# choyingw/SynergyNet

Measured on NVIDIA H100. Metric: faces/sec (120x120, batch 1024 per GPU, backbone + 3DMM params + 68 landmarks), higher is better.
Workload: dtype f32

## Files before the change

### synergynet_b200/csrc/kernels_fused.cuh

```cuda
#pragma once
#include "common.cuh"
#include "tc_common.cuh"

namespace syn {

constexpr int kFusedWorkerWarps = 8;
static_assert(kFusedWorkerWarps % 4 == 0, "worker warps form whole warpgroups");

__host__ __device__ constexpr int ceil_div_c(int a, int b) { return (a + b - 1) / b; }
__host__ __device__ constexpr int round_up_c(int a, int b) { return ceil_div_c(a, b) * b; }

template <int CIN_, int CHID_, int NC_, int COUT_, int W_, int STRIDE_, int RO_, int FACES_, bool RES_, bool STEM_,
          int WSTREAM_>
struct FusedCfg {
  static constexpr bool STEM = STEM_;
  static constexpr bool RES = RES_;
  static constexpr bool WSTREAM = WSTREAM_ > 0;
  static constexpr int CIN = CIN_;
  static constexpr int CIN_P = round_up_c(CIN_, 16);
  static constexpr int CHID = CHID_, NC = NC_, NCHUNK = CHID_ / NC_;
  static constexpr int COUT = COUT_, COUT_P = round_up_c(COUT_, 16);
  static constexpr int W = W_, STRIDE = STRIDE_, WO = (W_ - 1) / STRIDE_ + 1;
  static constexpr int RO = RO_, STRIPS = WO / RO_, FACES = FACES_;
  static constexpr int RWIN = (RO_ - 1) * STRIDE_ + 3;
  static constexpr int ROWS_MAX = (RWIN < W_ ? RWIN : W_);
  static constexpr int M1_MAX = FACES_ * ROWS_MAX * W_;
  static constexpr int MT1 = ceil_div_c(M1_MAX, 128);
  static constexpr int M2F = RO_ * WO;
  static constexpr int M2_MAX = FACES_ * M2F;
  static constexpr int MT2 = ceil_div_c(M2_MAX, 128);
  static constexpr int HS_COLS = W_ + 2;
  static constexpr int HS_FACE = RWIN * HS_COLS, HS_PIX = FACES_ * HS_FACE, HS_STRIDE = NC_ + 4;
  static constexpr int DWS = NC_ + 4;
  static constexpr int SLABS1 = ceil_div_c(M1_MAX, 64), SLABS2 = ceil_div_c(M2_MAX, 64);
  static constexpr int B3_BYTES = round_up_c(2 * COUT_P * 4, 128);
  static constexpr int W1_PLANE = NC_ * CIN_P * 2;
  static constexpr int W3_PLANE = COUT_P * NC_ * 2;
  static constexpr int DW_ROWS = 12;
  static constexpr int CH_W1 = 0, CH_W3 = 2 * W1_PLANE, CH_DW = CH_W3 + 2 * W3_PLANE;
  static constexpr int CHUNK_BYTES = round_up_c(CH_DW + DW_ROWS * DWS * 4, 128);
  static constexpr int W_BYTES = B3_BYTES + NCHUNK * CHUNK_BYTES;
  static constexpr int WSTAGES = WSTREAM_ > 0 ? WSTREAM_ : NCHUNK;
  static constexpr int A2_PLANE = MT2 * 128 * NC_ * 2;
  static constexpr int XA_TILE = 64 * CIN_P * 2, XA_PLANE = SLABS1 * XA_TILE;
  static constexpr int S_B3 = 0;
  static constexpr int S_WCH = S_B3 + B3_BYTES;
  static constexpr int S_XA = S_WCH + WSTAGES * CHUNK_BYTES;
  static constexpr int S_A2 = S_XA + 2 * XA_PLANE;
  static constexpr int S_H = S_A2 + 2 * A2_PLANE;
  static constexpr int IN_ROWS = 2 * ROWS_MAX + 1, IN_STRIDE = 120;
  static constexpr int S_IN = S_H + HS_PIX * HS_STRIDE * 4;
  static constexpr int S_TOTAL = S_IN + (STEM_ ? 3 * IN_ROWS * IN_STRIDE * 4 : 0);
  static constexpr int SMEM_BYTES = S_TOTAL + 1024;
  static_assert(CHID_ % NC_ == 0 && NC_ % 16 == 0, "hidden chunking");
  static_assert(WO % RO_ == 0, "strips must tile the output");
  static_assert(FACES_ == 1 || RO_ == WO, "multi-face tiles hold whole faces");
  static_assert(SMEM_BYTES <= 227 * 1024, "shared memory");
  static_assert(NC_ <= 256, "MMA N");
  static_assert(WSTREAM_ == 0 || (WSTREAM_ >= 2 && WSTREAM_ <= 4 && NCHUNK >= WSTREAM_), "weight ring");
};

struct FusedArgs {
  const float* x;
  const uint8_t* x_u8;
  const uint8_t* wimg;
  float* y;
  int batch;
  int split;
  int face_groups;
  int* err;
  int* sat;
  int border;
  int npass;
#ifdef SYN_FUSED_TRACE
  int trace_id;
#endif
};

#ifdef SYN_FUSED_TRACE
__device__ long long g_fused_trace[18 * 2 * 64 * 8];
#define SYN_TRACE(role, chunk, ev)                                                                        \
  do {                                                                                                    \
    if (trace_on) g_fused_trace[((p.trace_id * 2 + (role)) * 64 + (chunk)) * 8 + (ev)] = clock64();      \
  } while (0)
#else
#define SYN_TRACE(role, chunk, ev) do { } while (0)
#endif

template <int THREADS>
__device__ __forceinline__ void group_bar_sync(int grp) {
  switch (grp) {
    case 0: asm volatile("bar.sync 1, %0;" ::"n"(THREADS) : "memory"); break;
    case 1: asm volatile("bar.sync 2, %0;" ::"n"(THREADS) : "memory"); break;
    case 2: asm volatile("bar.sync 3, %0;" ::"n"(THREADS) : "memory"); break;
    default: asm volatile("bar.sync 4, %0;" ::"n"(THREADS) : "memory"); break;
  }
}

__host__ __device__ constexpr int fused_d2_pieces(int cout_p, int slabs, int nwg) {
  int s = 1;
  while (slabs * s < nwg && (cout_p / (2 * s)) % 8 == 0) s *= 2;
  return s;
}

template <int N, int KSTEPS, int NPASS>
__device__ __forceinline__ void fused_mma_group(float* acc, uint32_t d_hi, uint32_t a_lo, uint32_t a_plane, uint32_t a_kstep,
                                                uint32_t b_lo, uint32_t b_plane, uint32_t b_kstep, bool acc_in) {
  tc::wgmma_fence();
#pragma unroll
  for (int pass = 0; pass < NPASS; ++pass)
#pragma unroll
    for (int ks = 0; ks < KSTEPS; ++ks)
      tc::wgmma_f16<N>(acc, tc::desc64(d_hi, a_lo + (((pass == 2 ? a_plane : 0) + ks * a_kstep) >> 4)),
                       tc::desc64(d_hi, b_lo + (((pass == 1 ? b_plane : 0) + ks * b_kstep) >> 4)),
                       (acc_in || pass > 0 || ks > 0) ? 1u : 0u);
  tc::wgmma_commit();
}

template <class C>
__global__ void __launch_bounds__((kFusedWorkerWarps + 1) * 32, 1) fused_mbconv_kernel(const FusedArgs p) {
  constexpr int NWW = kFusedWorkerWarps;
  constexpr int NWT = NWW * 32;
  constexpr int NWG = NWW / 4;
  constexpr int NKG_ = C::NC / 8;
  constexpr int NG = 1;
  constexpr int WPG = NWW / NG, TPG = WPG * 32;
  constexpr int KPG = NKG_ / NG;
  constexpr int NSPL = fused_d2_pieces(C::COUT_P, C::SLABS2, NWG);
  constexpr int N2 = C::COUT_P / NSPL;
  constexpr int IPW = ceil_div_c(C::SLABS2 * NSPL, NWG);
  static_assert(N2 % 8 == 0 && N2 <= 256, "MMA N");
  using namespace tc;
  extern __shared__ __align__(1024) uint8_t smem_raw[];
  __shared__ __align__(8) uint64_t bar_w, bar_wfull[4], bar_wempty[4], bar_x, bar_in;

  uint8_t* smem = smem_raw + ((1024u - (smem_u32(smem_raw) & 1023u)) & 1023u);
  const int tid = threadIdx.x, warp = tid >> 5;
  const int row = tid & 127, wg = __shfl_sync(0xffffffffu, tid >> 7, 0);
  const int grp = warp / WPG;
  const int gtid = tid - grp * TPG;
  const int ntiles = p.face_groups * C::STRIPS;
  auto group_faces = [&](int fg, int& f0, int& nfaces) {
    if constexpr (C::FACES == 2) {
      if (fg < p.split) { f0 = 2 * fg; nfaces = 2; }
      else { f0 = 2 * p.split + (fg - p.split); nfaces = 1; }
    } else {
      f0 = fg * C::FACES;
      nfaces = min(C::FACES, p.batch - f0);
    }
  };

  asm volatile("griddepcontrol.launch_dependents;" ::: "memory");
  if (tid == 0) {
    mbar_init(smem_u32(&bar_w), 1);
    for (int i = 0; i < 4; ++i) {
      mbar_init(smem_u32(&bar_wfull[i]), 1);
      mbar_init(smem_u32(&bar_wempty[i]), NWT);
    }
    mbar_init(smem_u32(&bar_x), NWT);
    mbar_init(smem_u32(&bar_in), 1);
    fence_mbar_init();
  }
  if constexpr (C::STEM) {
    float* z = reinterpret_cast<float*>(smem_raw + ((1024u - (tc::smem_u32(smem_raw) & 1023u)) & 1023u) + C::S_IN);
    for (int i = threadIdx.x; i < 3 * C::IN_ROWS * C::IN_STRIDE / 4; i += blockDim.x)
      reinterpret_cast<float4*>(z)[i] = make_float4(0.f, 0.f, 0.f, 0.f);
    tc::fence_proxy_async_smem();
  }
  __syncthreads();

  uint8_t* sWch = smem + C::S_WCH;
  uint8_t* sXA = smem + C::S_XA;
  uint8_t* sA2 = smem + C::S_A2;
  float* sH = reinterpret_cast<float*>(smem + C::S_H);
  const float* sB3 = reinterpret_cast<const float*>(smem + C::S_B3);
  float* sIn = reinterpret_cast<float*>(smem + C::S_IN);

  if (warp < NWW) {
    for (int i = tid; i < C::HS_PIX * C::HS_STRIDE / 4; i += NWT)
      reinterpret_cast<float4*>(sH)[i] = make_float4(0.f, 0.f, 0.f, 0.f);
    mbar_wait(smem_u32(&bar_w), 0, p.err);
    uint32_t g = 0, n_in = 0;
    asm volatile("bar.sync 5, %0;" ::"n"(NWT) : "memory");
    const uint32_t d_hi = smem_desc_hi(128);
    constexpr uint32_t LBO_W1 = (C::NC / 8) * 128, LBO_W3 = (C::COUT_P / 8) * 128;

    constexpr int SPW = ceil_div_c(C::SLABS1, NWG);
    constexpr bool LATE_G1 = C::WSTREAM && C::WSTAGES == 2;
    auto issue_g1 = [&](bool on, float* acc, int s1, const uint8_t* wch) {
      if (on) {
        const uint32_t a_lo = smem_desc_lo(smem_u32(sXA + s1 * C::XA_TILE), 1024);
        const uint32_t w_lo = smem_desc_lo(smem_u32(wch + C::CH_W1), LBO_W1);
        if (p.npass == 1) fused_mma_group<C::NC, C::CIN_P / 16, 1>(acc, d_hi, a_lo, C::XA_PLANE, 2048, w_lo, C::W1_PLANE, 2 * LBO_W1, false);
        else fused_mma_group<C::NC, C::CIN_P / 16, 3>(acc, d_hi, a_lo, C::XA_PLANE, 2048, w_lo, C::W1_PLANE, 2 * LBO_W1, false);
      } else {
        wgmma_fence();
        wgmma_commit();
      }
    };

    auto prep = [&](int tile) {
      const int fg = tile / C::STRIPS, sp = tile - fg * C::STRIPS;
      int f0, nfaces;
      group_faces(fg, f0, nfaces);
      const int iy0 = sp * C::RO * C::STRIDE - 1;
      const int rf = max(iy0, 0), rl = min(iy0 + C::RWIN - 1, C::W - 1);
      const int ppf = (rl - rf + 1) * C::W;
      const int M1 = nfaces * ppf;
      const int mt1 = (M1 + 127) >> 7;
#ifdef SYN_FUSED_TRACE
      const bool trace_on = blockIdx.x == 0 && tile == 2 * (int)gridDim.x && tid == 0;
#endif
      SYN_TRACE(0, 62, 0);
      if constexpr (C::STEM) {
        const int iy_first = 2 * rf - 1, nin = 2 * (rl - rf + 1) + 1;
        if (p.x_u8 != nullptr) {
          for (int i = tid; i < 3 * nin * 30; i += NWT) {
            const int c4 = i % 30, r = (i / 30) % nin, ci = i / (30 * nin);
            const int iy = iy_first + r;
            float4 v = make_float4(0.f, 0.f, 0.f, 0.f);
            if (iy >= 0 && iy < kImg) {
              uchar4 u = *reinterpret_cast<const uchar4*>(p.x_u8 + ((size_t)(f0 * 3 + ci) * kImg + iy) * kImg + c4 * 4);
              if (p.border > 0) {
                const int col = c4 * 4;
                const bool row_out = iy < p.border || iy >= kImg - p.border;
                if (row_out || col < p.border || col >= kImg - p.border) u.x = 0;
                if (row_out || col + 1 < p.border || col + 1 >= kImg - p.border) u.y = 0;
                if (row_out || col + 2 < p.border || col + 2 >= kImg - p.border) u.z = 0;
                if (row_out || col + 3 < p.border || col + 3 >= kImg - p.border) u.w = 0;
              }
              v = make_float4(((float)u.x - 127.5f) / 128.0f, ((float)u.y - 127.5f) / 128.0f,
                              ((float)u.z - 127.5f) / 128.0f, ((float)u.w - 127.5f) / 128.0f);
            }
            *reinterpret_cast<float4*>(sIn + (ci * C::IN_ROWS + r) * C::IN_STRIDE + c4 * 4) = v;
          }
        } else {
          mbar_wait(smem_u32(&bar_in), n_in & 1, p.err);
          ++n_in;
          for (int r = 0; r < nin; ++r) {
            const int iy = iy_first + r;
            if (iy < 0 || iy >= kImg)
              for (int i = tid; i < 3 * 30; i += NWT)
                *reinterpret_cast<float4*>(sIn + ((i / 30) * C::IN_ROWS + r) * C::IN_STRIDE + (i % 30) * 4) =
                    make_float4(0.f, 0.f, 0.f, 0.f);
          }
        }
        SYN_TRACE(0, 62, 1);
        asm volatile("bar.sync 5, %0;" ::"n"(NWT) : "memory");
      }
      SYN_TRACE(0, 62, 2);
      {
        constexpr int KG = C::CIN_P / 8;
        constexpr int NXG = NWT / 64;
        constexpr int ITERS = (C::SLABS1 * KG + NXG - 1) / NXG;
        constexpr int PB = ITERS < 4 ? ITERS : 4;
        const int r64 = tid & 63, xg = tid >> 6;
        const int n_items = ((M1 + 63) >> 6) * KG;
        for (int e0 = xg; e0 < n_items; e0 += PB * NXG) {
          float v[PB][8];
          if constexpr (C::STEM) {
#pragma unroll
            for (int u = 0; u < PB; ++u) {
#pragma unroll
              for (int j = 0; j < 8; ++j) v[u][j] = 0.f;
              const int e = e0 + u * NXG;
              if (e >= n_items) continue;
              const int t = e / KG, kg = e - t * KG;
              const int mr = t * 64 + r64;
              if (mr < M1) {
                const int yl = mr / C::W, xx = mr - yl * C::W;
                const float* base = sIn + (2 * yl) * C::IN_STRIDE + 2 * xx - 1;
#pragma unroll
                for (int kgc = 0; kgc < KG; ++kgc)
                  if (kg == kgc) {
#pragma unroll
                    for (int j = 0; j < 8; ++j) {
                      const int k = kgc * 8 + j;
                      if (k < 27) {
                        const int ci = k / 9, ky = (k % 9) / 3, kx = k % 3;
                        if (kx > 0 || xx > 0) v[u][j] = base[(ci * C::IN_ROWS + ky) * C::IN_STRIDE + kx];
                      }
                    }
                  }
              }
            }
          } else {
            float4 qa[PB], qb[PB];
            bool ok[PB];
#pragma unroll
            for (int u = 0; u < PB; ++u) {
              const int e = min(e0 + u * NXG, n_items - 1);
              const int t = e / KG, kg = e - t * KG;
              const int m = t * 64 + r64;
              ok[u] = (e0 + u * NXG < n_items) && (m < M1) && (kg * 8 < C::CIN);
              const int mc = min(m, M1 - 1), kgc = min(kg, (C::CIN - 1) / 8);
              const int f = (C::FACES > 1) ? mc / ppf : 0;
              const int mr = mc - f * ppf;
              const float* src = p.x + ((size_t)((f0 + f) * C::W + rf) * C::W + mr) * C::CIN + kgc * 8;
              qa[u] = __ldg(reinterpret_cast<const float4*>(src));
              qb[u] = __ldg(reinterpret_cast<const float4*>(src + 4));
            }
            if (e0 == xg) SYN_TRACE(0, 62, 5);
#pragma unroll
            for (int u = 0; u < PB; ++u) {
              v[u][0] = ok[u] ? qa[u].x : 0.f; v[u][1] = ok[u] ? qa[u].y : 0.f; v[u][2] = ok[u] ? qa[u].z : 0.f; v[u][3] = ok[u] ? qa[u].w : 0.f;
              v[u][4] = ok[u] ? qb[u].x : 0.f; v[u][5] = ok[u] ? qb[u].y : 0.f; v[u][6] = ok[u] ? qb[u].z : 0.f; v[u][7] = ok[u] ? qb[u].w : 0.f;
            }
          }
#pragma unroll
          for (int u = 0; u < PB; ++u) {
            const int e = e0 + u * NXG;
            if (e < n_items) {
              const int t = e / KG, kg = e - t * KG;
              uint32_t h[4], l[4];
              float vmax = 0.f;
#pragma unroll
              for (int j = 0; j < 8; ++j) vmax = fmaxf(vmax, fabsf(v[u][j]));
              if (vmax * kActScale > 60000.f) *p.sat = 1;
#pragma unroll
              for (int j = 0; j < 4; ++j) split2_f16(v[u][2 * j] * kActScale, v[u][2 * j + 1] * kActScale, h[j], l[j]);
              uint8_t* xa = sXA + t * C::XA_TILE + (r64 >> 3) * 128 + kg * 1024 + (r64 & 7) * 16;
              *reinterpret_cast<uint4*>(xa) = make_uint4(h[0], h[1], h[2], h[3]);
              *reinterpret_cast<uint4*>(xa + C::XA_PLANE) = make_uint4(l[0], l[1], l[2], l[3]);
              if (e == xg) SYN_TRACE(0, 62, 6);
            }
          }
          if (e0 == xg) SYN_TRACE(0, 62, 7);
        }
      }
      SYN_TRACE(0, 62, 3);
      fence_proxy_async_smem();
      mbar_arrive(smem_u32(&bar_x));
      SYN_TRACE(0, 62, 4);

    };
    auto prefetch_x = [&](int tile) {
      if constexpr (!C::STEM) {
        if (tile >= ntiles) return;
        const int fg = tile / C::STRIPS, sp = tile - fg * C::STRIPS;
        int f0, nfaces;
        group_faces(fg, f0, nfaces);
        const int iy0 = sp * C::RO * C::STRIDE - 1;
        const int rf = max(iy0, 0), rl = min(iy0 + C::RWIN - 1, C::W - 1);
        const char* base = reinterpret_cast<const char*>(p.x + ((size_t)(f0 * C::W + rf) * C::W) * C::CIN);
        const int bytes = (C::FACES > 1 ? nfaces * C::W * C::W : (rl - rf + 1) * C::W) * C::CIN * 4;
        for (int o = tid * 128; o < bytes; o += NWT * 128)
          asm volatile("prefetch.global.L2 [%0];" ::"l"(base + o));
      }
    };
    asm volatile("griddepcontrol.wait;" ::: "memory");
    if ((int)blockIdx.x < ntiles) prep(blockIdx.x);
    prefetch_x(blockIdx.x + gridDim.x);

    for (int tile = blockIdx.x; tile < ntiles; tile += gridDim.x) {
      const int fg = tile / C::STRIPS, sp = tile - fg * C::STRIPS;
      int f0, nfaces;
      group_faces(fg, f0, nfaces);
      const int oy0 = sp * C::RO;
      const int iy0 = oy0 * C::STRIDE - 1;
      const int rf = max(iy0, 0), rl = min(iy0 + C::RWIN - 1, C::W - 1);
      const int ppf = (rl - rf + 1) * C::W;
#ifdef SYN_FUSED_TRACE
      const bool trace_on = blockIdx.x == 0 && tile == (int)gridDim.x && tid == 0;
#endif
      SYN_TRACE(0, 63, 0);
      const int M1 = nfaces * ppf;
      const int mt1 = (M1 + 127) >> 7;
      const int M2 = nfaces * C::M2F;
      const int mt2 = (M2 + 127) >> 7;

      const int slabs1 = (M1 + 63) >> 6;
      float acc1[2][C::NC / 2];
      float acc2[IPW][N2 / 2];
      auto chunk_slot = [&](uint32_t gc, int c) -> const uint8_t* {
        const int slot = C::WSTREAM ? (int)(gc % C::WSTAGES) : c;
        if constexpr (C::WSTREAM) mbar_wait(smem_u32(&bar_wfull[slot]), (gc / C::WSTAGES) & 1, p.err);
        return sWch + slot * C::CHUNK_BYTES;
      };
      auto gemm1_epi1 = [&](int c, const uint8_t* wch) {
        const float* dwc = reinterpret_cast<const float*>(wch + C::CH_DW);
        const float sc1 = dwc[11 * C::DWS];
        const float* b1 = dwc + 10 * C::DWS;
#pragma unroll
        for (int j = 0; j < SPW; ++j) {
          const int s1 = wg + j * NWG;
          if (j + 1 < SPW) issue_g1(s1 + NWG < slabs1, acc1[(j + 1) & 1], s1 + NWG, wch);
          if (j + 1 < SPW) wgmma_wait<1>();
          else wgmma_wait<0>();
          if (s1 >= slabs1) continue;
          const float* acc = acc1[j & 1];
#pragma unroll
          for (int h = 0; h < 2; ++h) {
            const int m = 64 * s1 + acc_row(row, 2 * h);
            if (m < M1) {
              const int f = (C::FACES > 1) ? m / ppf : 0;
              const int mr = m - f * ppf;
              const int yl = mr / C::W, xx = mr - yl * C::W;
              float* hrow = sH + (size_t)(f * C::HS_FACE + (rf - iy0 + yl) * C::HS_COLS + xx + 1) * C::HS_STRIDE;
#pragma unroll
              for (int q = 0; q < C::NC / 8; ++q) {
                const int i = 4 * q + 2 * h, j0 = acc_col(row, i);
                const float2 bq = *reinterpret_cast<const float2*>(b1 + j0);
                *reinterpret_cast<float2*>(hrow + j0) =
                    make_float2(__saturatef(fmaf(acc[i], sc1, bq.x)), __saturatef(fmaf(acc[i + 1], sc1, bq.y)));
              }
            }
          }
        }
        wgmma_wait<0>();
        SYN_TRACE(0, c, 3);
      };
      {
        SYN_TRACE(0, 0, 0);
        const uint8_t* w0 = chunk_slot(g, 0);
        group_bar_sync<TPG>(grp);
        SYN_TRACE(0, 0, 1);
        if constexpr (C::STRIPS > 1) {
          constexpr int CQ = KPG * 2;
          if (iy0 < 0)
            for (int i = gtid; i < C::HS_COLS * CQ; i += TPG)
              *reinterpret_cast<float4*>(sH + (size_t)(i / CQ) * C::HS_STRIDE + grp * KPG * 8 + (i % CQ) * 4) =
                  make_float4(0.f, 0.f, 0.f, 0.f);
          if (iy0 + C::RWIN - 1 > C::W - 1)
            for (int i = gtid; i < C::HS_COLS * CQ; i += TPG)
              *reinterpret_cast<float4*>(sH + (size_t)((C::RWIN - 1) * C::HS_COLS + i / CQ) * C::HS_STRIDE +
                                         grp * KPG * 8 + (i % CQ) * 4) = make_float4(0.f, 0.f, 0.f, 0.f);
        }
        issue_g1(wg < slabs1, acc1[0], wg, w0);
        gemm1_epi1(0, w0);
      }
      for (int c = 0; c < C::NCHUNK; ++c, ++g) {
        const int slot = C::WSTREAM ? (int)(g % C::WSTAGES) : c;
        const uint8_t* wch = sWch + slot * C::CHUNK_BYTES;
        const float* dwc = reinterpret_cast<const float*>(wch + C::CH_DW);
        group_bar_sync<TPG>(grp);
        SYN_TRACE(0, c, 4);
        const bool more = c + 1 < C::NCHUNK;
        const uint8_t* wn = wch;
        if constexpr (!LATE_G1) {
          if (more) wn = chunk_slot(g + 1, c + 1);
          issue_g1(more && wg < slabs1, acc1[0], wg, wn);
        }
        if constexpr (C::STRIDE == 1 && ((C::WO >= 15 && C::WO <= 30) || C::WO == 8)) {
          constexpr int XL = (C::WO >= 15) ? 8 : 4, YL = 8 / XL;
          constexpr int CPR = (C::WO + 1) / 2, XG2 = (CPR + XL - 1) / XL, RP2 = (C::RO + 1) / 2;
          constexpr int RPU = (RP2 + YL - 1) / YL, UPK = RPU * XG2;
          const int l8 = tid & 7, qh = (tid >> 3) & 1;
          const int lx = l8 % XL, ly = l8 / XL;
          const bool mir = (l8 & 4) != 0;
          const int units = KPG * nfaces * UPK;
          for (int u = gtid >> 4; u < units; u += TPG / 16) {
            const int kgl = u / (nfaces * UPK), r1 = u - kgl * (nfaces * UPK);
            const int f = r1 / UPK, r2 = r1 - f * UPK;
            const int rpu = r2 / XG2, xg = r2 - rpu * XG2;
            const int kg = grp * KPG + kgl, j0 = kg * 8 + qh * 4;
            const int ox = 2 * (xg * XL + lx), oy = 2 * (rpu * YL + ly);
            if (ox >= C::WO || oy >= C::RO) continue;
            const bool two = (oy + 1 < C::RO);
            const float* wq = dwc + j0;
            float2 w[3][3][2];
#pragma unroll
            for (int ky = 0; ky < 3; ++ky)
#pragma unroll
              for (int kl = 0; kl < 3; ++kl) {
                const float4 t4 = *reinterpret_cast<const float4*>(wq + (ky * 3 + (mir ? 2 - kl : kl)) * C::DWS);
                w[ky][kl][0] = make_float2(t4.x, t4.y); w[ky][kl][1] = make_float2(t4.z, t4.w);
              }
            float2 acc[2][2][2];
            {
              const float4 b4 = *reinterpret_cast<const float4*>(wq + 9 * C::DWS);
#pragma unroll
              for (int ro = 0; ro < 2; ++ro)
#pragma unroll
                for (int a = 0; a < 2; ++a) { acc[ro][a][0] = make_float2(b4.x, b4.y); acc[ro][a][1] = make_float2(b4.z, b4.w); }
            }
            const float* hb = sH + (size_t)(f * C::HS_FACE + oy * C::HS_COLS + ox + (mir ? 3 : 0)) * C::HS_STRIDE + j0;
            const int cstep = mir ? -C::HS_STRIDE : C::HS_STRIDE;
#pragma unroll
            for (int ic = 0; ic < 4; ++ic) {
              float2 d[4][2];
#pragma unroll
              for (int r = 0; r < 4; ++r) {
                if (r == 3 && !two) continue;
                const float4 t4 = *reinterpret_cast<const float4*>(hb + r * (C::HS_COLS * C::HS_STRIDE) + ic * cstep);
                d[r][0] = make_float2(t4.x, t4.y); d[r][1] = make_float2(t4.z, t4.w);
              }
#pragma unroll
              for (int a = 0; a < 2; ++a) {
                const int kl = ic - a;
                if (kl < 0 || kl > 2) continue;
#pragma unroll
                for (int ky = 0; ky < 3; ++ky) {
#pragma unroll
                  for (int j = 0; j < 2; ++j) acc[0][a][j] = ffma2(d[ky][j], w[ky][kl][j], acc[0][a][j]);
                  if (two) {
#pragma unroll
                    for (int j = 0; j < 2; ++j) acc[1][a][j] = ffma2(d[ky + 1][j], w[ky][kl][j], acc[1][a][j]);
                  }
                }
              }
            }
            constexpr float kOut = 6.0f * kActScale;
#pragma unroll
            for (int ro = 0; ro < 2; ++ro) {
              if (ro == 1 && !two) continue;
#pragma unroll
              for (int a = 0; a < 2; ++a) {
                const int col = ox + (mir ? 1 - a : a);
                if (col >= C::WO) continue;
                const int m2 = f * C::M2F + (oy + ro) * C::WO + col;
                uint32_t h0, l0, h1, l1;
                split2_f16<false>(__saturatef(acc[ro][a][0].x) * kOut, __saturatef(acc[ro][a][0].y) * kOut, h0, l0);
                split2_f16<false>(__saturatef(acc[ro][a][1].x) * kOut, __saturatef(acc[ro][a][1].y) * kOut, h1, l1);
                uint8_t* dst = sA2 + (m2 >> 7) * (128 * C::NC * 2) + ((m2 & 127) >> 3) * 128 + kg * 2048 + (m2 & 7) * 16 + qh * 8;
                *reinterpret_cast<uint2*>(dst) = make_uint2(h0, h1);
                *reinterpret_cast<uint2*>(dst + C::A2_PLANE) = make_uint2(l0, l1);
              }
            }
          }
        } else
        {
          constexpr int NKG = C::NC / 8;
          constexpr int GX = (C::WO >= 8) ? 8 : 4, GY = 8 / GX;
          constexpr int XG = (C::WO + GX - 1) / GX;
          constexpr int RPI = (4 * C::FACES * ((C::RO + 1) / 2) * ((C::WO + GX - 1) / GX) * GX * NKG <= NWT) ? 1 : 2;
          constexpr int RP = (C::RO + RPI - 1) / RPI, RPG = (RP + GY - 1) / GY;
          constexpr int PER_FACE = XG * RPG;
          constexpr int NR = (RPI - 1) * C::STRIDE + 3;
          const int per_kg = nfaces * PER_FACE;
          const int l8 = tid & 7, lx = l8 % GX, ly = l8 / GX;
          const bool swz = (C::STRIDE == 2) && (l8 & 4);
          const int q0 = swz ? 4 : 0, q1 = 4 - q0;
          {
            const int kg_end = (grp + 1) * KPG;
            int kg = grp * KPG, it = gtid >> 3;
            while (it >= per_kg && kg < kg_end) { it -= per_kg; ++kg; }
            while (kg < kg_end) {
              const int f = it / PER_FACE, r2 = it - f * PER_FACE;
              const int rpg = r2 / XG, xg = r2 - rpg * XG;
              const int ox = xg * GX + lx, oy = (RPI == 2) ? 2 * (rpg * GY + ly) : rpg + RPG * ly;
              if (ox < C::WO && oy < C::RO) {
                const float* wbase = dwc + kg * 8;
                const float* h0 = sH + (size_t)(f * C::HS_FACE + (oy * C::STRIDE) * C::HS_COLS + ox * C::STRIDE) * C::HS_STRIDE + kg * 8;
                const bool two = (RPI == 2) && (oy + 1 < C::RO);
                float2 acc0[4], acc1[4];
                {
                  const float4 a = *reinterpret_cast<const float4*>(wbase + 9 * C::DWS + q0);
                  const float4 e = *reinterpret_cast<const float4*>(wbase + 9 * C::DWS + q1);
                  acc0[0] = make_float2(a.x, a.y); acc0[1] = make_float2(a.z, a.w); acc0[2] = make_float2(e.x, e.y); acc0[3] = make_float2(e.z, e.w);
  #pragma unroll
                  for (int j = 0; j < 4; ++j) acc1[j] = acc0[j];
                }
  #pragma unroll
                for (int dx = 0; dx < 3; ++dx) {
                  float2 w[3][4];
  #pragma unroll
                  for (int dy = 0; dy < 3; ++dy) {
                    const float4 a = *reinterpret_cast<const float4*>(wbase + (dy * 3 + dx) * C::DWS + q0);
                    const float4 e = *reinterpret_cast<const float4*>(wbase + (dy * 3 + dx) * C::DWS + q1);
                    w[dy][0] = make_float2(a.x, a.y); w[dy][1] = make_float2(a.z, a.w);
                    w[dy][2] = make_float2(e.x, e.y); w[dy][3] = make_float2(e.z, e.w);
                  }
  #pragma unroll
                  for (int wr = 0; wr < NR; ++wr) {
                    if (wr >= 3 && !two) continue;
                    const float* hp = h0 + (wr * C::HS_COLS + dx) * C::HS_STRIDE;
                    const float4 a = *reinterpret_cast<const float4*>(hp + q0);
                    const float4 e = *reinterpret_cast<const float4*>(hp + q1);
                    const float2 d[4] = {make_float2(a.x, a.y), make_float2(a.z, a.w), make_float2(e.x, e.y), make_float2(e.z, e.w)};
                    if (wr < 3) {
  #pragma unroll
                      for (int j = 0; j < 4; ++j) acc0[j] = ffma2(d[j], w[wr][j], acc0[j]);
                    }
                    if (RPI == 2 && wr >= C::STRIDE) {
  #pragma unroll
                      for (int j = 0; j < 4; ++j) acc1[j] = ffma2(d[j], w[wr - C::STRIDE][j], acc1[j]);
                    }
                  }
                }
                constexpr float kOut = 6.0f * kActScale;
                const int m2 = f * C::M2F + oy * C::WO + ox;
                {
                  uint32_t h[4], l[4];
  #pragma unroll
                  for (int j = 0; j < 4; ++j)
                    split2_f16<false>(__saturatef(acc0[j].x) * kOut, __saturatef(acc0[j].y) * kOut, h[j], l[j]);
                  uint8_t* dst = sA2 + (m2 >> 7) * (128 * C::NC * 2) + ((m2 & 127) >> 3) * 128 + kg * 2048 + (m2 & 7) * 16;
                  *reinterpret_cast<uint4*>(dst) = swz ? make_uint4(h[2], h[3], h[0], h[1]) : make_uint4(h[0], h[1], h[2], h[3]);
                  *reinterpret_cast<uint4*>(dst + C::A2_PLANE) = swz ? make_uint4(l[2], l[3], l[0], l[1]) : make_uint4(l[0], l[1], l[2], l[3]);
                }
                if (two) {
                  const int m3 = m2 + C::WO;
                  uint32_t h[4], l[4];
  #pragma unroll
                  for (int j = 0; j < 4; ++j)
                    split2_f16<false>(__saturatef(acc1[j].x) * kOut, __saturatef(acc1[j].y) * kOut, h[j], l[j]);
                  uint8_t* dst = sA2 + (m3 >> 7) * (128 * C::NC * 2) + ((m3 & 127) >> 3) * 128 + kg * 2048 + (m3 & 7) * 16;
                  *reinterpret_cast<uint4*>(dst) = swz ? make_uint4(h[2], h[3], h[0], h[1]) : make_uint4(h[0], h[1], h[2], h[3]);
                  *reinterpret_cast<uint4*>(dst + C::A2_PLANE) = swz ? make_uint4(l[2], l[3], l[0], l[1]) : make_uint4(l[0], l[1], l[2], l[3]);
                }
              }
              it += TPG / 8;
              while (it >= per_kg && kg < kg_end) { it -= per_kg; ++kg; }
            }
          }
        }
        SYN_TRACE(0, c, 5);
        if constexpr (LATE_G1) {
          if (more) wn = chunk_slot(g + 1, c + 1);
          issue_g1(more && wg < slabs1, acc1[0], wg, wn);
        }
        fence_proxy_async_smem();
        group_bar_sync<TPG>(grp);
        {
          const uint32_t w_lo = smem_desc_lo(smem_u32(wch + C::CH_W3), LBO_W3);
          const int items2 = ((M2 + 63) >> 6) * NSPL;
#pragma unroll
          for (int u = 0; u < IPW; ++u) {
            const int it = wg + u * NWG;
            if (it < items2) {
              const int s2 = it / NSPL, pc = it - s2 * NSPL;
              const uint32_t a_lo = smem_desc_lo(smem_u32(sA2 + (s2 >> 1) * (128 * C::NC * 2)) + (s2 & 1) * 1024, 2048);
              const uint32_t b_lo = w_lo + ((pc * (N2 / 8) * 128) >> 4);
              if (p.npass == 1) fused_mma_group<N2, C::NC / 16, 1>(acc2[u], d_hi, a_lo, C::A2_PLANE, 4096, b_lo, C::W3_PLANE, 2 * LBO_W3, c > 0);
              else fused_mma_group<N2, C::NC / 16, 3>(acc2[u], d_hi, a_lo, C::A2_PLANE, 4096, b_lo, C::W3_PLANE, 2 * LBO_W3, c > 0);
            } else {
              wgmma_fence();
              wgmma_commit();
            }
          }
        }
        wgmma_wait<0>();
        if constexpr (C::WSTREAM) mbar_arrive(smem_u32(&bar_wempty[slot]));
        SYN_TRACE(0, c, 6);
        if (more) {
          SYN_TRACE(0, c + 1, 0);
          SYN_TRACE(0, c + 1, 1);
          gemm1_epi1(c + 1, wn);
        }
      }
      SYN_TRACE(0, 63, 1);

      if (tile + (int)gridDim.x < ntiles) prep(tile + gridDim.x);
      prefetch_x(tile + 2 * (int)gridDim.x);
      SYN_TRACE(0, 63, 2);
      auto out_pixel = [&](int m2) -> int {
        if (m2 >= M2) return -1;
        return m2;
      };
      const int items2 = ((M2 + 63) >> 6) * NSPL;
#pragma unroll
      for (int u = 0; u < IPW; ++u) {
        const int it = wg + u * NWG;
        if (it >= items2) break;
        const int s2 = it / NSPL, pc = it - s2 * NSPL;
#pragma unroll
        for (int h = 0; h < 2; ++h) {
          const int pix = out_pixel(64 * s2 + acc_row(row, 2 * h));
          if (pix < 0) continue;
          float* orow = p.y + ((size_t)(f0 * C::WO + oy0) * C::WO + pix) * C::COUT;
          const float* xrow = p.x + ((size_t)(f0 * C::W + oy0) * C::W + pix) * C::CIN;
          float2 res[N2 / 8];
          if constexpr (C::RES) {
#pragma unroll
            for (int q = 0; q < N2 / 8; ++q) {
              const int j = pc * N2 + acc_col(row, 4 * q);
              res[q] = j < C::COUT ? __ldg(reinterpret_cast<const float2*>(xrow + j)) : make_float2(0.f, 0.f);
            }
          }
#pragma unroll
          for (int q = 0; q < N2 / 8; ++q) {
            const int i = 4 * q + 2 * h, j = pc * N2 + acc_col(row, i);
            if (j < C::COUT) {
              const float2 bb = *reinterpret_cast<const float2*>(sB3 + j);
              const float2 sc = *reinterpret_cast<const float2*>(sB3 + C::COUT_P + j);
              float2 o = make_float2(fmaf(acc2[u][i], sc.x, bb.x), fmaf(acc2[u][i + 1], sc.y, bb.y));
              if constexpr (C::RES) { o.x += res[q].x; o.y += res[q].y; }
              *reinterpret_cast<float2*>(orow + j) = o;
            }
          }
        }
      }
      SYN_TRACE(0, 63, 4);
    }
  } else if (warp == NWW) {
    const int my_tiles = (ntiles > (int)blockIdx.x) ? (ntiles - 1 - (int)blockIdx.x) / (int)gridDim.x + 1 : 0;
    const uint32_t total_chunks = (uint32_t)my_tiles * C::NCHUNK;
    auto load_chunk = [&](uint32_t gi) {
      const uint32_t slot = gi % C::WSTAGES, c = gi % C::NCHUNK;
      mbar_expect_tx(smem_u32(&bar_wfull[slot]), C::CHUNK_BYTES);
      bulk_g2s(smem_u32(sWch + slot * C::CHUNK_BYTES), p.wimg + C::B3_BYTES + (size_t)c * C::CHUNK_BYTES, C::CHUNK_BYTES,
               smem_u32(&bar_wfull[slot]));
    };
    if (elect_one()) {
      if constexpr (C::WSTREAM) {
        mbar_expect_tx(smem_u32(&bar_w), C::B3_BYTES);
        bulk_g2s(smem_u32(smem + C::S_B3), p.wimg, C::B3_BYTES, smem_u32(&bar_w));
        for (uint32_t k = 0; k < (uint32_t)C::WSTAGES; ++k)
          if (total_chunks > k) load_chunk(k);
      } else {
        mbar_expect_tx(smem_u32(&bar_w), C::W_BYTES);
        bulk_g2s(smem_u32(smem + C::S_B3), p.wimg, C::W_BYTES, smem_u32(&bar_w));
      }
    }
    __syncwarp();
    if constexpr (C::WSTREAM) {
      for (uint32_t gi = C::WSTAGES; gi < total_chunks; ++gi) {
        mbar_wait(smem_u32(&bar_wempty[gi % C::WSTAGES]), (gi / C::WSTAGES - 1) & 1, p.err);
        if (elect_one()) load_chunk(gi);
        __syncwarp();
      }
    }
    if constexpr (C::STEM) {
      auto stage_rows = [&](int tile) {
        if (p.x_u8 != nullptr || tile >= ntiles) return;
        if (!elect_one()) return;
        const int fgq = tile / C::STRIPS, spq = tile - fgq * C::STRIPS;
        const int iy0q = spq * C::RO * C::STRIDE - 1;
        const int rfq = max(iy0q, 0), rlq = min(iy0q + C::RWIN - 1, C::W - 1);
        const int iy_first = 2 * rfq - 1, nin = 2 * (rlq - rfq + 1) + 1;
        const int r_lo = (iy_first < 0) ? -iy_first : 0;
        const int r_hi = min(nin - 1, kImg - 1 - iy_first);
        const uint32_t bytes = (uint32_t)(r_hi - r_lo + 1) * kImg * 4;
        mbar_expect_tx(smem_u32(&bar_in), 3 * bytes);
        for (int ci = 0; ci < 3; ++ci)
          bulk_g2s(smem_u32(sIn + (ci * C::IN_ROWS + r_lo) * C::IN_STRIDE),
                   p.x + ((size_t)(fgq * 3 + ci) * kImg + iy_first + r_lo) * kImg, bytes, smem_u32(&bar_in));
      };
      asm volatile("griddepcontrol.wait;" ::: "memory");
      stage_rows(blockIdx.x);
      __syncwarp();
      uint32_t n_x = 0;
      for (int tile = blockIdx.x; p.x_u8 == nullptr && tile < ntiles; tile += gridDim.x) {
        mbar_wait(smem_u32(&bar_x), n_x & 1, p.err);
        ++n_x;
        stage_rows(tile + gridDim.x);
        __syncwarp();
      }
    }
  }
}

template <class C>
inline void fused_tile_plan(int batch, int sms, int& split, int& face_groups) {
  if constexpr (C::FACES == 2) {
    const int full = batch / 2, odd = batch & 1, rem = full % sms;
    split = (2 * rem + odd <= sms) ? full - rem : full;
    face_groups = split + (batch - 2 * split);
  } else {
    split = 0;
    face_groups = (batch + C::FACES - 1) / C::FACES;
  }
}

using FusedStemB1 = FusedCfg<27, 32, 32, 16, 60, 1, 6, 1, false, true, 0>;
using FusedB2 = FusedCfg<16, 96, 32, 24, 60, 2, 6, 1, false, false, 0>;
using FusedB3 = FusedCfg<24, 144, 48, 24, 30, 1, 6, 1, true, false, 0>;
using FusedB4 = FusedCfg<24, 144, 16, 32, 30, 2, 5, 1, false, false, 0>;
using FusedB56 = FusedCfg<32, 192, 64, 32, 15, 1, 5, 1, true, false, 0>;
using FusedB7 = FusedCfg<32, 192, 64, 64, 15, 2, 8, 1, false, false, 0>;
using FusedB8 = FusedCfg<64, 384, 64, 64, 8, 1, 8, 2, true, false, 3>;
using FusedB11 = FusedCfg<64, 384, 64, 96, 8, 1, 8, 2, false, false, 2>;
using FusedB12 = FusedCfg<96, 576, 32, 96, 8, 1, 8, 2, true, false, 3>;
using FusedB14 = FusedCfg<96, 576, 32, 160, 8, 2, 4, 2, false, false, 3>;
using FusedB15 = FusedCfg<160, 960, 32, 160, 4, 1, 4, 4, true, false, 3>;
using FusedB17 = FusedCfg<160, 960, 32, 320, 4, 1, 4, 4, false, false, 2>;

}
```

Before: 240,900.

## Carry halo rows between consecutive strips in fused stem kernel to skip recompute

For the stem configuration, each CTA now takes a contiguous run of tiles instead of a grid-strided set, so consecutive strips of the same face land on the same CTA. The two overlapping hidden-activation halo rows from the previous strip are moved in place in shared memory, and the next strip's expand GEMM starts two rows lower, avoiding recomputing those rows. It also widens the depthwise fast path's WO range. In exchange it adds extra shared-memory copies and synchronisation dependencies, and contiguous scheduling may change load balance and prefetch behaviour.

Result: faster. 245,600, median of 6 (+1.9%).

```diff
diff --git a/synergynet_b200/csrc/kernels_fused.cuh b/synergynet_b200/csrc/kernels_fused.cuh
--- a/synergynet_b200/csrc/kernels_fused.cuh
+++ b/synergynet_b200/csrc/kernels_fused.cuh
@@ -52,9 +52,12 @@
   static constexpr int S_IN = S_H + HS_PIX * HS_STRIDE * 4;
   static constexpr int S_TOTAL = S_IN + (STEM_ ? 3 * IN_ROWS * IN_STRIDE * 4 : 0);
   static constexpr int SMEM_BYTES = S_TOTAL + 1024;
+  static constexpr bool CARRY = STEM_;
   static_assert(CHID_ % NC_ == 0 && NC_ % 16 == 0, "hidden chunking");
   static_assert(WO % RO_ == 0, "strips must tile the output");
   static_assert(FACES_ == 1 || RO_ == WO, "multi-face tiles hold whole faces");
+  static_assert(!CARRY || (FACES_ == 1 && STRIPS > 1 && RWIN == RO_ + 2 && NCHUNK == 1),
+                "a carried strip computes the RO rows below two rows moved in place in its one-chunk window");
   static_assert(SMEM_BYTES <= 227 * 1024, "shared memory");
   static_assert(NC_ <= 256, "MMA N");
   static_assert(WSTREAM_ == 0 || (WSTREAM_ >= 2 && WSTREAM_ <= 4 && NCHUNK >= WSTREAM_), "weight ring");
@@ -148,6 +151,16 @@
       f0 = fg * C::FACES;
       nfaces = min(C::FACES, p.batch - f0);
     }
+  };
+  const int run = ntiles / (int)gridDim.x, run_rem = ntiles % (int)gridDim.x, cta = blockIdx.x;
+  const int t_first = C::CARRY ? cta * run + min(cta, run_rem) : cta;
+  const int t_end = C::CARRY ? t_first + run + (cta < run_rem ? 1 : 0) : ntiles;
+  const int t_step = C::CARRY ? 1 : (int)gridDim.x;
+  auto carried = [&](int tile) { return C::CARRY && tile != t_first && tile % C::STRIPS != 0; };
+  auto tile_rows = [&](int tile, int& iy0, int& rf, int& rl) {
+    iy0 = (tile % C::STRIPS) * C::RO * C::STRIDE - 1;
+    rf = carried(tile) ? iy0 + 2 : max(iy0, 0);
+    rl = min(iy0 + C::RWIN - 1, C::W - 1);
   };
 
   asm volatile("griddepcontrol.launch_dependents;" ::: "memory");
@@ -200,16 +213,14 @@
     };
 
     auto prep = [&](int tile) {
-      const int fg = tile / C::STRIPS, sp = tile - fg * C::STRIPS;
       int f0, nfaces;
-      group_faces(fg, f0, nfaces);
-      const int iy0 = sp * C::RO * C::STRIDE - 1;
-      const int rf = max(iy0, 0), rl = min(iy0 + C::RWIN - 1, C::W - 1);
+      group_faces(tile / C::STRIPS, f0, nfaces);
+      int iy0, rf, rl;
+      tile_rows(tile, iy0, rf, rl);
       const int ppf = (rl - rf + 1) * C::W;
       const int M1 = nfaces * ppf;
-      const int mt1 = (M1 + 127) >> 7;
 #ifdef SYN_FUSED_TRACE
-      const bool trace_on = blockIdx.x == 0 && tile == 2 * (int)gridDim.x && tid == 0;
+      const bool trace_on = blockIdx.x == 0 && tile == t_first + 2 * t_step && tid == 0;
 #endif
       SYN_TRACE(0, 62, 0);
       if constexpr (C::STEM) {
@@ -336,12 +347,11 @@
     };
     auto prefetch_x = [&](int tile) {
       if constexpr (!C::STEM) {
-        if (tile >= ntiles) return;
-        const int fg = tile / C::STRIPS, sp = tile - fg * C::STRIPS;
+        if (tile >= t_end) return;
         int f0, nfaces;
-        group_faces(fg, f0, nfaces);
-        const int iy0 = sp * C::RO * C::STRIDE - 1;
-        const int rf = max(iy0, 0), rl = min(iy0 + C::RWIN - 1, C::W - 1);
+        group_faces(tile / C::STRIPS, f0, nfaces);
+        int iy0, rf, rl;
+        tile_rows(tile, iy0, rf, rl);
         const char* base = reinterpret_cast<const char*>(p.x + ((size_t)(f0 * C::W + rf) * C::W) * C::CIN);
         const int bytes = (C::FACES > 1 ? nfaces * C::W * C::W : (rl - rf + 1) * C::W) * C::CIN * 4;
         for (int o = tid * 128; o < bytes; o += NWT * 128)
@@ -349,19 +359,20 @@
       }
     };
     asm volatile("griddepcontrol.wait;" ::: "memory");
-    if ((int)blockIdx.x < ntiles) prep(blockIdx.x);
-    prefetch_x(blockIdx.x + gridDim.x);
-
-    for (int tile = blockIdx.x; tile < ntiles; tile += gridDim.x) {
+    if (t_first < t_end) prep(t_first);
+    prefetch_x(t_first + t_step);
+
+    for (int tile = t_first; tile < t_end; tile += t_step) {
       const int fg = tile / C::STRIPS, sp = tile - fg * C::STRIPS;
       int f0, nfaces;
       group_faces(fg, f0, nfaces);
       const int oy0 = sp * C::RO;
-      const int iy0 = oy0 * C::STRIDE - 1;
-      const int rf = max(iy0, 0), rl = min(iy0 + C::RWIN - 1, C::W - 1);
+      int iy0, rf, rl;
+      tile_rows(tile, iy0, rf, rl);
       const int ppf = (rl - rf + 1) * C::W;
+      const bool keep = tile + t_step < t_end && carried(tile + t_step);
 #ifdef SYN_FUSED_TRACE
-      const bool trace_on = blockIdx.x == 0 && tile == (int)gridDim.x && tid == 0;
+      const bool trace_on = blockIdx.x == 0 && tile == t_first + t_step && tid == 0;
 #endif
       SYN_TRACE(0, 63, 0);
       const int M1 = nfaces * ppf;
@@ -441,7 +452,7 @@
           if (more) wn = chunk_slot(g + 1, c + 1);
           issue_g1(more && wg < slabs1, acc1[0], wg, wn);
         }
-        if constexpr (C::STRIDE == 1 && ((C::WO >= 15 && C::WO <= 30) || C::WO == 8)) {
+        if constexpr (C::STRIDE == 1 && ((C::WO >= 15 && C::WO <= 60) || C::WO == 8)) {
           constexpr int XL = (C::WO >= 15) ? 8 : 4, YL = 8 / XL;
           constexpr int CPR = (C::WO + 1) / 2, XG2 = (CPR + XL - 1) / XL, RP2 = (C::RO + 1) / 2;
           constexpr int RPU = (RP2 + YL - 1) / YL, UPK = RPU * XG2;
@@ -630,6 +641,16 @@
             }
           }
         }
+        if constexpr (C::CARRY) {
+          if (keep) {
+            constexpr int Q = C::NC / 4;
+            for (int i = tid; i < 2 * C::W * Q; i += NWT) {
+              const int px = i / Q, r = px / C::W;
+              float* win = sH + (size_t)(r * C::HS_COLS + px - r * C::W + 1) * C::HS_STRIDE + (i - px * Q) * 4;
+              *reinterpret_cast<float4*>(win) = *reinterpret_cast<const float4*>(win + C::RO * C::HS_COLS * C::HS_STRIDE);
+            }
+          }
+        }
         wgmma_wait<0>();
         if constexpr (C::WSTREAM) mbar_arrive(smem_u32(&bar_wempty[slot]));
         SYN_TRACE(0, c, 6);
@@ -641,8 +662,8 @@
       }
       SYN_TRACE(0, 63, 1);
 
-      if (tile + (int)gridDim.x < ntiles) prep(tile + gridDim.x);
-      prefetch_x(tile + 2 * (int)gridDim.x);
+      if (tile + t_step < t_end) prep(tile + t_step);
+      prefetch_x(tile + 2 * t_step);
       SYN_TRACE(0, 63, 2);
       auto out_pixel = [&](int m2) -> int {
         if (m2 >= M2) return -1;
@@ -684,7 +705,7 @@
       SYN_TRACE(0, 63, 4);
     }
   } else if (warp == NWW) {
-    const int my_tiles = (ntiles > (int)blockIdx.x) ? (ntiles - 1 - (int)blockIdx.x) / (int)gridDim.x + 1 : 0;
+    const int my_tiles = (t_end > t_first) ? (t_end - 1 - t_first) / t_step + 1 : 0;
     const uint32_t total_chunks = (uint32_t)my_tiles * C::NCHUNK;
     auto load_chunk = [&](uint32_t gi) {
       const uint32_t slot = gi % C::WSTAGES, c = gi % C::NCHUNK;
@@ -713,11 +734,11 @@
     }
     if constexpr (C::STEM) {
       auto stage_rows = [&](int tile) {
-        if (p.x_u8 != nullptr || tile >= ntiles) return;
+        if (p.x_u8 != nullptr || tile >= t_end) return;
         if (!elect_one()) return;
-        const int fgq = tile / C::STRIPS, spq = tile - fgq * C::STRIPS;
-        const int iy0q = spq * C::RO * C::STRIDE - 1;
-        const int rfq = max(iy0q, 0), rlq = min(iy0q + C::RWIN - 1, C::W - 1);
+        const int fgq = tile / C::STRIPS;
+        int iy0q, rfq, rlq;
+        tile_rows(tile, iy0q, rfq, rlq);
         const int iy_first = 2 * rfq - 1, nin = 2 * (rlq - rfq + 1) + 1;
         const int r_lo = (iy_first < 0) ? -iy_first : 0;
         const int r_hi = min(nin - 1, kImg - 1 - iy_first);
@@ -728,13 +749,13 @@
                    p.x + ((size_t)(fgq * 3 + ci) * kImg + iy_first + r_lo) * kImg, bytes, smem_u32(&bar_in));
       };
       asm volatile("griddepcontrol.wait;" ::: "memory");
-      stage_rows(blockIdx.x);
+      stage_rows(t_first);
       __syncwarp();
       uint32_t n_x = 0;
-      for (int tile = blockIdx.x; p.x_u8 == nullptr && tile < ntiles; tile += gridDim.x) {
+      for (int tile = t_first; p.x_u8 == nullptr && tile < t_end; tile += t_step) {
         mbar_wait(smem_u32(&bar_x), n_x & 1, p.err);
         ++n_x;
-        stage_rows(tile + gridDim.x);
+        stage_rows(tile + t_step);
         __syncwarp();
       }
     }
```
